# martinber/noaa-apt

Measured on AMD Instinct MI355X. Metric: Msamples/sec WAV->APT-line decode, higher is better.
Workload: dtype f32; 1 GPU; synthetic 48000 Hz APT recording, 600 s (28800000 samples) per GPU, profile=standard: resample 13/50 (959 taps) -> AM envelope -> 37-tap low-pass -> sync correlation + peak picker -> 1198 rows x 2080 px; parallelism=1 GPU(s), 16 independent recordings per GPU and step, no collectives, recordings_per_call=16, mode=strict, rows=1198, n_sync=1199, input_resident_in_hbm=True, distinct_inputs_round_robin=16

## Files before the change

noaa_apt_amd/csrc/apt_capi.hip:

```cpp
#include <cstdio>
#include <cstdlib>
#include <cstring>
#include <memory>
#include <string>

#include "apt_capi_util.hpp"
#include "apt_session.hpp"

namespace {

using namespace apt::capi;

using PlanPtr = std::unique_ptr<aptgpu_plan, apt::capi::PlanDeleter>;


apt::Signal download(const float *d, size_t n, hipStream_t s)
{
    apt::Signal h(n);
    if (n) {
        apt::hip_check(hipMemcpyAsync(h.data(), d, n * sizeof(float), hipMemcpyDeviceToHost, s),
                       "hipMemcpyAsync D2H");
        apt::hip_check(hipStreamSynchronize(s), "hipStreamSynchronize");
    }
    return h;
// ... 189 lines not shown
        (void)hipSetDevice(plan->device);
        plan->sync_all();
        plan->sync_all();
        auto v = plan->timer.collect(plan->stream);
        *n_out = v.size();
        for (size_t i = 0; i < v.size() && i < cap && out; ++i) out[i] = v[i];
        return APTGPU_OK;
    } catch (const Error &) {
        return APTGPU_ERR_HIP;
    }
}

int aptgpu_plan_read_internal(aptgpu_plan *plan, int i, const char *name, void *host_out,
                              size_t bytes, size_t *size_out)
{
    if (!plan || !name || i < 0 || static_cast<size_t>(i) >= plan->last_slots.size())
        return APTGPU_ERR_INVALID;
    aptgpu_plan::Slot &sl = plan->slot_of(i);
    const void *src = nullptr;
    size_t size = 0;
    const std::string n(name);
    if (n == "inv_sinphi") {
        if (size_out) *size_out = sizeof(float);
        if (host_out && bytes >= sizeof(float)) std::memcpy(host_out, &plan->inv_sinphi, sizeof(float));
        return APTGPU_OK;
    }
    if (n == "filtered") { src = sl.filtered.ptr; size = sl.filtered.count * sizeof(float); }
    else if (n == "correlation") { src = sl.correlation.ptr; size = sl.correlation.count * sizeof(float); }
    else if (n == "group_max") { src = sl.gm.ptr; size = sl.gm.count * sizeof(apt::gpu::GroupMax); }
    else if (n == "terminal_words") { src = sl.words.ptr; size = sl.words.count * sizeof(uint64_t); }
    else if (n == "peaks") { src = sl.peaks.ptr; size = sl.peaks.count * sizeof(uint32_t); }
    else if (n == "picker_flags") { src = sl.flags.ptr; size = sl.flags.count * sizeof(uint32_t); }
    else if (n == "eqfloat_thresholds") {
        src = sl.eqfloat_ws.ptr ? apt::gpu::eqfloat_ws_thresholds(sl.eqfloat_ws.ptr) : nullptr;
        size = sl.eqfloat_ws.ptr ? 2 * 255 * sizeof(uint32_t) : 0;
    }
    else return APTGPU_ERR_INVALID;
    if (size_out) *size_out = size;
    (void)hipSetDevice(plan->device);
    try {
        plan->sync_all();
    } catch (const Error &) {
        return APTGPU_ERR_HIP;
    }
    const size_t take = bytes < size ? bytes : size;
    if (take && host_out && src &&
        hipMemcpy(host_out, src, take, hipMemcpyDeviceToHost) != hipSuccess)
        return APTGPU_ERR_HIP;
    return APTGPU_OK;
}

}

namespace apt::capi {

int decode_host(const aptgpu_context *ctx_in, const aptgpu_settings *settings, const float *signal,
                const uint8_t *wav_data, const apt::WavInfo *wav, size_t n, uint32_t input_rate_hz, int sync,
                float **rows_out, size_t *n_out, aptgpu_stats *stats, char *err, size_t err_cap)
{
    *rows_out = nullptr;
// ... 488 lines not shown
```

noaa_apt_amd/csrc/apt_kernels.hpp:

```cpp
#pragma once

#include <hip/hip_runtime.h>

#include <cstdint>

namespace apt::gpu {

struct Result {
    int32_t status;
    int32_t reason;
    uint32_t n_rows;
    uint32_t n_sync;
    uint64_t work_len;
    uint64_t n_out;
};

struct ImageResult {
    int32_t status;
    int32_t reason;
    uint32_t height;
    uint32_t telemetry_row;
    float low, high;
    float telemetry_quality;
    int32_t channel_a, channel_b;
// ... 48 lines not shown
                      uint32_t ntaps, uint32_t l, uint32_t m, float *out, uint64_t w);
uint32_t f16taps_pairs_per_phase(uint32_t l, uint32_t ntaps);
float f16taps_pack(uint32_t l, const float *coeff, uint32_t ntaps, uint16_t *table);
void resample_f16taps(hipStream_t s, const float *x, uint64_t n, const uint16_t *table, uint32_t ntaps,
                      uint32_t l, uint32_t m, float unscale, float *out, uint64_t w);
void fir_decimate(hipStream_t s, const float *x, uint64_t n, const float *coeff, uint32_t ntaps,
                  uint32_t m, float *out, uint64_t n_out);
void demodulate(hipStream_t s, const float *x, uint64_t n, float cosphi2, float sinphi, float *out);
void correlate(hipStream_t s, const float *f, uint64_t n_corr, uint32_t pw, float *corr);
void terminals(hipStream_t s, const float *corr, uint64_t n_corr, uint32_t md, uint64_t *bits);
void orbit_walk(hipStream_t s, const uint64_t *bits, const float *corr, uint64_t n_corr, uint64_t work_len,
                uint32_t spr, uint32_t md, uint32_t *peaks, uint32_t peaks_cap, Result *res);
void gather_rows(hipStream_t s, const float *f, const uint32_t *peaks, Result *res,
                 uint32_t spr, uint32_t pw, bool raw, float *rows, uint32_t rows_cap);
void gather_rows_call(hipStream_t s, const CallArgs &call, const SlotPtrs *d_slots, uint32_t spr, uint32_t pw,
                      uint32_t max_rows_cap, const LaunchSwitches &sw = LaunchSwitches{});

void nosync_rows_call(hipStream_t s, const CallArgs &call, const SlotPtrs *d_slots, uint32_t spr, uint32_t m2, uint64_t max_w);

bool fused_supported(uint32_t l, uint32_t m, uint32_t t1, uint32_t t2, uint32_t pw);
uint32_t fused_group_size(uint32_t l);
bool fused_takes_pcm16(uint32_t l, uint32_t m);
uint32_t fused_tap_table_floats(uint32_t l, uint32_t m, uint32_t t1, int ch);
void fused_branch_taps(uint32_t l, uint32_t m, const float *coeff, uint32_t t1, int ch, float *hs, uint32_t t1_layout = 0);
uint32_t fused_pad_t1(uint32_t l, uint32_t m, uint32_t t1, uint32_t t2, uint32_t pw);
uint32_t fused_pad_t2(uint32_t l, uint32_t m, uint32_t t2, uint32_t pw);
uint32_t fused_phase_pad_t2(uint32_t t2, uint32_t pw);
int fused_chunk_of(uint32_t m, bool fast);
void fused_lowpass_pairs(const float *h2, uint32_t t2, float *h2p);
uint32_t fused_f16_table_dwords(uint32_t l, uint32_t m, uint32_t t1);
float fused_f16_branch_taps(uint32_t l, uint32_t m, const float *coeff, uint32_t t1, uint32_t *table);
bool fused_f16_supported(uint32_t l, uint32_t m, uint32_t t1, uint32_t t2, uint32_t pw);
float fused_gm_slack(uint32_t pw, float scale = 1.f);
// ... 96 lines not shown
```

noaa_apt_amd/csrc/apt_kernels_fused_any_impl.hpp:

```cpp
#pragma once

#include "apt_kernels_fused_any_launch.hpp"
#include "apt_envelope.hpp"
#include "apt_sync_corr.hpp"

#include <atomic>
#include <type_traits>

#pragma clang fp contract(off)

namespace apt::gpu {


namespace {


constexpr int kGS = 52;
constexpr float kNegInfAny = -__builtin_huge_valf();


typedef float f2 __attribute__((ext_vector_type(2)));

template <int KPT>
__host__ __device__ constexpr int pad_ofs(int e)
// ... 220 lines not shown
#pragma unroll
                for (int jj = 0; jj < KPT; ++jj) {
                    if (j0 + jj < G.t2) {
                        const float hj = h2[j0 + jj];
#pragma unroll
                        for (int u = 0; u < KPT; ++u) acc[u] = acc[u] + win[KPT + u - jj] * hj;
                    }
                }
            }
#pragma unroll
            for (int u = 0; u < KPT; ++u) A[P(b0) + u] = acc[u];
        }
    }
    __syncthreads();

    for (uint32_t q = tid * 4; q < G.own; q += NTHR * 4) {
        const uint64_t k = static_cast<uint64_t>(o0) + q;
        const float *src = A + P(static_cast<int>(G.pre + q));
        if (k + 3 < w) {
            *reinterpret_cast<float4 *>(f_out + k) = make_float4(src[0], src[1], src[2], src[3]);
        } else {
            for (int e = 0; e < 4; ++e)
                if (k + e < w) f_out[k + e] = src[e];
        }
    }
    if (gm_out == nullptr) return;

    const uint32_t pw = PWC > 0 ? static_cast<uint32_t>(PWC) : G.pulse / 2u;
    const uint32_t pulse = 2u * pw;
    float *AB = X;
    {
        const int b0 = static_cast<int>(G.pre) + tid * KPT;
        if (b0 < static_cast<int>(G.pre + G.own + 36u * pw)) {
            float bs[KPT];
            if constexpr (PWC > 0) {
                constexpr int NW = KPT + 2 * PWC - 1;
                float wv[NW];
                const float *src = A + P(b0);
// ... 116 lines not shown
```

noaa_apt_amd/csrc/apt_kernels_fused_impl.hpp:

```cpp
#pragma once

#include "apt_kernels_fused_launch.hpp"
#include "apt_envelope.hpp"
#include "apt_sync_corr.hpp"

#include <hip/hip_runtime.h>

#include <algorithm>
#include <atomic>
#include <cmath>
#include <cstdlib>
#include <type_traits>

#pragma clang fp contract(off)

#define APT_S1(n) "s" #n
#define APT_S8_(a, b, c, d, e, f, g, h) APT_S1(a), APT_S1(b), APT_S1(c), APT_S1(d), APT_S1(e), APT_S1(f), APT_S1(g), APT_S1(h)
#define APT_S8(n) APT_S8_X(n)
#define APT_S16(n) APT_S16_X(n)
#define APT_S8_X(n) APT_S8_##n
#define APT_S16_X(n) APT_S16_##n
#define APT_S8_52 APT_S8_(52, 53, 54, 55, 56, 57, 58, 59)
#define APT_S16_36 APT_S8_(36, 37, 38, 39, 40, 41, 42, 43), APT_S8_(44, 45, 46, 47, 48, 49, 50, 51)
#define APT_S16_64 APT_S8_(64, 65, 66, 67, 68, 69, 70, 71), APT_S8_(72, 73, 74, 75, 76, 77, 78, 79)
// ... 1440 lines not shown
                for (int b = 0; b < L; ++b) {
                    const int qi = tid * L + b - static_cast<int>(j);
                    if (kt + b > static_cast<int>(j) && qi >= 0) f[b] = f[b] + Q[qi] * hj;
                }
            }
#pragma unroll
            for (int b = 0; b < L; ++b) P[tid * L + b] = f[b];
            __syncthreads();
        }
    }
    APT_MARK("END f_to_lds");
    if constexpr (APT_FUSED_STOP == 4) return;
    uint32_t slot_late = call.rec[ri].slot;
    asm volatile("" : "+s"(slot_late));
    float *__restrict__ f_out = slots[slot_late].f;
    if (interior) {
        APT_MARK("BEGIN f_store");
        typedef char __attribute__((address_space(1))) *gchar_wptr;
        typedef f4 __attribute__((address_space(1))) *gfloat4_wptr;
        gchar_wptr sb = (gchar_wptr)(f_out + o0);
        const uint32_t voff = static_cast<uint32_t>(tid) * 16u;
#pragma unroll
        for (int e = 0; e * kFusedThreads * 4 < Gm::OWN_K; ++e) {
            const int q = (tid + e * kFusedThreads) * 4;
            if (q < Gm::OWN_K) {
                const float *src = P + Gm::PRE_K + q;
                *(gfloat4_wptr)(sb + voff) = (f4){src[0], src[1], src[2], src[3]};
            }
            sb += kFusedThreads * 16;
            asm volatile("" : "+s"(sb));
        }
        APT_MARK("END f_store");
    } else {
        float *ft = f_out + o0;
        for (int q = tid * 4; q < Gm::OWN_K; q += kFusedThreads * 4) {
            if (Gm::PRE_K + q + 3 < k_hi) {
                const float *src = P + Gm::PRE_K + q;
                *reinterpret_cast<float4 *>(ft + q) = make_float4(src[0], src[1], src[2], src[3]);
            } else {
                for (int e = 0; e < 4; ++e)
                    if (Gm::PRE_K + q + e < k_hi) ft[q + e] = P[Gm::PRE_K + q + e];
            }
        }
    }
    if constexpr (APT_FUSED_STOP == 5) return;
    if (want_gm) {
        GroupMax *__restrict__ gm_out = slots[slot_late].gm;
        constexpr int PUL = 2 * PW;
        static_assert(Gm::GS == 4 * L, "a group is four threads' samples");
        float ab_mine = 0.f;
        {
            APT_MARK("BEGIN pulse_sums");
            int fofs = tid * L;
            int qofs4 = Gm::D_OFF + tid * L;
            int fofs_odd = fofs + 1;
            asm volatile("" : "+v"(fofs), "+v"(fofs_odd), "+v"(qofs4));
            constexpr int NFW = L + PUL - 1;
// ... 283 lines not shown
```

noaa_apt_amd/csrc/apt_kernels_generic.hip:

```cpp
#include "apt_kernels.hpp"
#include "apt_envelope.hpp"

#include <hip/hip_runtime.h>

#include <cstdlib>

#include <cmath>
#include <cstring>
#include <map>
#include <mutex>
#include <tuple>

#pragma clang fp contract(off)

namespace apt::gpu {

namespace {

constexpr int kBlock = 256;

inline unsigned grid_for(uint64_t n, unsigned block, unsigned cap = 256u * 32u)
{
    uint64_t g = (n + block - 1) / block;
    if (g > cap) g = cap;
// ... 233 lines not shown
        res->n_rows = static_cast<uint32_t>(fit - last_fit);
        res->work_len = work_len;
        res->n_out = (fit - last_fit) * 2080u;
        if (len < 5) {
            res->status = 1;
            res->reason = 2;
            res->n_rows = 0;
            res->n_out = 0;
        } else {
            res->status = 0;
            res->reason = 0;
        }
    }
}

__device__ __forceinline__ void gather_rows_body(const float *__restrict__ f, const uint32_t *__restrict__ peaks,
                                                 Result *__restrict__ res, uint32_t spr, uint32_t pw, int raw,
                                                 float *__restrict__ rows, uint32_t rows_cap)
{
    uint32_t n_rows = __hip_atomic_load(&res->n_rows, __ATOMIC_RELAXED, __HIP_MEMORY_SCOPE_AGENT);
    const uint32_t px_per_row = spr / pw;
    if (n_rows > rows_cap) {
        n_rows = rows_cap;
        if (blockIdx.x == 0 && blockIdx.y == 0 && threadIdx.x == 0) {
            __hip_atomic_store(&res->n_rows, rows_cap, __ATOMIC_RELAXED, __HIP_MEMORY_SCOPE_AGENT);
            res->n_out = static_cast<uint64_t>(rows_cap) * px_per_row;
            res->reason = 4;
        }
    }
    const bool quads = (px_per_row & 3u) == 0 && (reinterpret_cast<uintptr_t>(rows) & 15u) == 0;
    for (uint32_t r = blockIdx.y; r < n_rows; r += gridDim.y) {
        const float *src = f + peaks[r];
        float *dst = rows + static_cast<uint64_t>(r) * px_per_row;
        if (quads) {
            for (uint32_t k = blockIdx.x * blockDim.x + threadIdx.x; k < px_per_row / 4u; k += gridDim.x * blockDim.x) {
                const float *p4 = src + static_cast<uint64_t>(4u * k) * pw;
                float4 v = make_float4(p4[0], p4[pw], p4[2u * pw], p4[3u * pw]);
                if (!raw) {
                    v.x = __fadd_rn(0.f, __fmul_rn(v.x, 1.f));
                    v.y = __fadd_rn(0.f, __fmul_rn(v.y, 1.f));
                    v.z = __fadd_rn(0.f, __fmul_rn(v.z, 1.f));
                    v.w = __fadd_rn(0.f, __fmul_rn(v.w, 1.f));
                    if (r == 0 && k == 0) v.x = 0.f;
                }
                *reinterpret_cast<float4 *>(dst + 4u * k) = v;
            }
            continue;
        }
        for (uint32_t c = blockIdx.x * blockDim.x + threadIdx.x; c < px_per_row;
             c += gridDim.x * blockDim.x) {
            float v = src[static_cast<uint64_t>(c) * pw];
            if (!raw) {
                v = __fadd_rn(0.f, __fmul_rn(v, 1.f));
                if (r == 0 && c == 0) v = 0.f;
            }
            dst[c] = v;
        }
    }
}

__global__ void __launch_bounds__(kBlock)
k_gather_rows(const float *__restrict__ f, const uint32_t *__restrict__ peaks,
              Result *__restrict__ res, uint32_t spr, uint32_t pw, int raw,
              float *__restrict__ rows, uint32_t rows_cap)
{
    gather_rows_body(f, peaks, res, spr, pw, raw, rows, rows_cap);
}

__global__ void __launch_bounds__(kBlock)
k_gather_rows_call(const CallArgs call, const SlotPtrs *__restrict__ slots, uint32_t spr, uint32_t pw)
{
    const RecArgs rec = call.rec[blockIdx.z];
    const SlotPtrs sp = slots[rec.slot];
    gather_rows_body(sp.f, sp.peaks, sp.res, spr, pw, 0, rec.rows, rec.rows_cap);
}

template <uint32_t QPR>
__global__ void __launch_bounds__(kBlock)
k_gather_rows_flat(const CallArgs call, const SlotPtrs *__restrict__ slots, uint32_t spr, uint32_t pw)
{
    const RecArgs rec = call.rec[blockIdx.y];
    const SlotPtrs sp = slots[rec.slot];
    Result *__restrict__ res = sp.res;
    uint32_t n_rows = __hip_atomic_load(&res->n_rows, __ATOMIC_RELAXED, __HIP_MEMORY_SCOPE_AGENT);
    if (n_rows > rec.rows_cap) {
        n_rows = rec.rows_cap;
        if (blockIdx.x == 0 && threadIdx.x == 0) {
            __hip_atomic_store(&res->n_rows, rec.rows_cap, __ATOMIC_RELAXED, __HIP_MEMORY_SCOPE_AGENT);
            res->n_out = static_cast<uint64_t>(rec.rows_cap) * (QPR * 4u);
            res->reason = 4;
        }
    }
    const float *__restrict__ f = sp.f;
    const uint32_t *__restrict__ peaks = sp.peaks;
    float *__restrict__ rows = rec.rows;
    const uint32_t total = n_rows * QPR;
    for (uint32_t q = blockIdx.x * kBlock + threadIdx.x; q < total; q += gridDim.x * kBlock) {
        const uint32_t r = q / QPR, k = q - r * QPR;
        const float *p4 = f + peaks[r] + static_cast<uint64_t>(4u * k) * pw;
        float4 v = make_float4(p4[0], p4[pw], p4[2u * pw], p4[3u * pw]);
        v.x = __fadd_rn(0.f, __fmul_rn(v.x, 1.f));
        v.y = __fadd_rn(0.f, __fmul_rn(v.y, 1.f));
        v.z = __fadd_rn(0.f, __fmul_rn(v.z, 1.f));
        v.w = __fadd_rn(0.f, __fmul_rn(v.w, 1.f));
        if (q == 0) v.x = 0.f;
        *reinterpret_cast<float4 *>(rows + static_cast<uint64_t>(q) * 4u) = v;
    }
}

__global__ void k_set_result(Result *res, Result value) { *res = value; }

__global__ void __launch_bounds__(kBlock)
k_nosync_rows_call(const CallArgs call, const SlotPtrs *__restrict__ slots, uint32_t spr, uint32_t m2)
{
    const RecArgs rec = call.rec[blockIdx.y];
    const float *__restrict__ f = slots[rec.slot].f;
    const uint64_t aligned = rec.w / spr * spr;
    uint64_t n_out = aligned / m2;
    if (n_out > rec.rows_cap) n_out = rec.rows_cap;
    const uint64_t stride = static_cast<uint64_t>(gridDim.x) * blockDim.x;
    for (uint64_t k = static_cast<uint64_t>(blockIdx.x) * blockDim.x + threadIdx.x; k < n_out; k += stride) {
        const uint64_t i = k * m2;
        rec.rows[k] = i < 1 ? 0.f : __fadd_rn(0.f, __fmul_rn(f[i], 1.f));
    }
    if (blockIdx.x == 0 && threadIdx.x == 0)
        *slots[rec.slot].res = Result{0 , 0, static_cast<uint32_t>(n_out / 2080u), 0, rec.w, n_out};
}

}

void set_result(hipStream_t s, Result *res, Result value)
{
    hipLaunchKernelGGL(k_set_result, dim3(1), dim3(1), 0, s, res, value);
}

void nosync_rows_call(hipStream_t s, const CallArgs &call, const SlotPtrs *d_slots, uint32_t spr, uint32_t m2, uint64_t max_w)
{
    if (call.count == 0 || spr == 0 || m2 == 0) return;
    const uint64_t n = max_w / m2 + 1;
    hipLaunchKernelGGL(k_nosync_rows_call, dim3(grid_for(n, kBlock), call.count), dim3(kBlock), 0, s, call, d_slots, spr, m2);
}

void resample_generic(hipStream_t s, const float *x, uint64_t n, const float *coeff,
                      uint32_t ntaps, uint32_t l, uint32_t m, float *out, uint64_t w)
{
    if (w == 0) return;
    const uint32_t jlim = 2 * ((ntaps - 1) / 2) + 1;
    hipLaunchKernelGGL(k_resample_generic, dim3(grid_for(w, kBlock)), dim3(kBlock), 0, s, x, n,
                       coeff, jlim, l, m, out, w);
}

uint32_t f16taps_pairs_per_phase(uint32_t l, uint32_t ntaps) { return ((ntaps + l - 1) / l + 1) / 2; }

float f16taps_pack(uint32_t l, const float *coeff, uint32_t ntaps, uint16_t *table)
{
// ... 72 lines not shown
    LaunchSwitches sw;
    if (const char *e = std::getenv("APTGPU_GATHER_ITERS")) sw.gather_iters = std::atoi(e);
    if (const char *e = std::getenv("APTGPU_WORDS_DPP")) sw.words_dpp = e[0] != '0';
    if (const char *e = std::getenv("APTGPU_ORBIT_LDS")) sw.orbit_lds = e[0] != '0';
    if (const char *e = std::getenv("APTGPU_ORBIT_THREADS")) sw.orbit_threads = std::atoi(e);
    if (const char *e = std::getenv("APTGPU_ORBIT_ALG")) sw.orbit_alg = e[0] == '0' ? 0 : 1;
    if (const char *e = std::getenv("APTGPU_GM_SLACK_SCALE")) {
        const float v = std::strtof(e, nullptr);
        if (v >= 1.f) sw.gm_slack_scale = v;
    }
    if (const char *e = std::getenv("APTGPU_FUSED_LDS_PAD")) sw.fused_lds_pad = std::max(0, std::atoi(e));
    return sw;
}

void gather_rows_call(hipStream_t s, const CallArgs &call, const SlotPtrs *d_slots, uint32_t spr, uint32_t pw,
                      uint32_t max_rows_cap, const LaunchSwitches &sw)
{
    if (call.count == 0) return;
    {
        const int iters = sw.gather_iters;
        bool aligned = true;
        for (uint32_t i = 0; i < call.count; ++i) aligned = aligned && (reinterpret_cast<uintptr_t>(call.rec[i].rows) & 15u) == 0;
        if (iters > 0 && spr / pw == 2080u && spr % pw == 0 && aligned && max_rows_cap > 0) {
            const uint64_t quads = static_cast<uint64_t>(max_rows_cap < 32768u ? max_rows_cap : 32768u) * 520u;
            const uint64_t per_wg = static_cast<uint64_t>(kBlock) * static_cast<uint64_t>(iters);
            const unsigned gx = static_cast<unsigned>((quads + per_wg - 1) / per_wg);
            hipLaunchKernelGGL(k_gather_rows_flat<520u>, dim3(gx ? gx : 1, call.count), dim3(kBlock), 0, s, call, d_slots, spr, pw);
            return;
        }
    }
    const unsigned rows_cap = max_rows_cap < 32768u ? max_rows_cap : 32768u;
    const unsigned gy = max_rows_cap == 0 ? 1u : (rows_cap + 7u) / 8u;
    const unsigned gx = (spr / pw + 4 * kBlock - 1) / (4 * kBlock);
    hipLaunchKernelGGL(k_gather_rows_call, dim3(gx ? gx : 1, gy, call.count), dim3(kBlock), 0, s, call, d_slots,
                       spr, pw);
}

void gather_rows(hipStream_t s, const float *f, const uint32_t *peaks, Result *res,
                 uint32_t spr, uint32_t pw, bool raw, float *rows, uint32_t rows_cap)
{
    const unsigned gy = rows_cap == 0 ? 1u : (rows_cap < 4096u ? rows_cap : 4096u);
    const unsigned gx = (spr / pw + 4 * kBlock - 1) / (4 * kBlock);
    hipLaunchKernelGGL(k_gather_rows, dim3(gx ? gx : 1, gy), dim3(kBlock), 0, s, f, peaks, res, spr,
                       pw, raw ? 1 : 0, rows, rows_cap);
}


__global__ void __launch_bounds__(256) k_verify_fast_divide(float c, float rc, uint32_t *bad)
{
    const uint32_t i = blockIdx.x * 256u + threadIdx.x;
// ... 75 lines not shown
```

noaa_apt_amd/csrc/apt_kernels_sync.hip:

```cpp
#include "apt_kernels.hpp"
#include "apt_sync_corr.hpp"

#include <hip/hip_runtime.h>

#include <atomic>

#include <cstdlib>
#include <type_traits>

namespace apt::gpu {

namespace {

constexpr int GS = 52;
constexpr uint64_t kGroupMask = (1ull << GS) - 1;
constexpr float kNegInf = -__builtin_huge_valf();

__global__ void __launch_bounds__(256)
k_group_max(const float *__restrict__ corr, uint64_t n_corr, GroupMax *__restrict__ gm, uint32_t ng)
{
    const uint32_t g = blockIdx.x * blockDim.x + threadIdx.x;
    if (g >= ng) return;
    const uint64_t base = static_cast<uint64_t>(g) * GS;
    float mx = kNegInf;
// ... 167 lines not shown
        const float wm = fmaxf(a[q + 1], a[q + 1 + W - K]);
        s_wm[q] = wm;
        if (g < static_cast<int64_t>(ng) && !(wm > s_hi[q])) s_cand[atomicAdd(&s_ncand, 1u)] = static_cast<uint16_t>(q);
        __syncthreads();
    }

    const uint32_t ncand = s_ncand;
    constexpr int kBatch = NL > 0 ? 4 : 1;
    constexpr int NLR = NL > 0 ? NL : 1;
    constexpr uint16_t kDeferred = 0x8000u;
    float *wa = s_win + static_cast<size_t>(wave) * wlen;
    const uint32_t wneed = GS + 38u * pw - 1u;
    auto eval_group = [&](uint64_t base, bool on) -> float {
        for (uint32_t t = lane; t < wlen; t += 64) {
            const uint64_t j = base + t;
            wa[t] = (t < wneed && j < w) ? fsig[j] : 0.f;
        }
        __builtin_amdgcn_wave_barrier();
        const float v = nodes_eval_window<NL, PWC>(wa, on, lane, pw, fast);
        __builtin_amdgcn_wave_barrier();
        return v;
    };
    auto settle = [&](auto exact_tag, int q, float cv, float c2v, bool in_v) -> bool {
        constexpr bool EXACT = decltype(exact_tag)::value;
        const uint64_t base = static_cast<uint64_t>(gw0 + q) * GS;
        const bool in2 = in_v && base + lane + md < n_corr;
        if (in_v && gw0 + q == 0 && lane == 0 && !(cv > 0.f)) cv = 0.f;
        const unsigned long long nanword = __ballot(in_v && cv != cv) & kGroupMask;
        if (cv != cv) cv = kNegInf;
        float sfx_ex;
        if constexpr (DPP) {
// ... 82 lines not shown
            qv[e] = (ci < ncand) ? s_cand[ci] : -1;
            const int64_t g = gw0 + (qv[e] < 0 ? 0 : qv[e]);
            const uint64_t i = static_cast<uint64_t>(g) * GS + lane;
            inv[e] = qv[e] >= 0 && lane < GS && i < n_corr;
            cv[e] = kNegInf;
            c2v[e] = kNegInf;
            if (corr != nullptr) {
                if (inv[e]) {
                    cv[e] = corr[i];
                    if (i + md < n_corr) c2v[e] = corr[i + md];
                }
            } else if constexpr (NL > 0) {
#pragma unroll
                for (int t = 0; t < NL; ++t) {
                    const uint64_t j = static_cast<uint64_t>(g) * GS + lane + 64u * t;
                    fa[e][t] = (qv[e] >= 0 && lane + 64u * t < wneed && j < w) ? fsig[j] : 0.f;
                }
            }
        }
#pragma unroll
        for (int e = 0; e < kBatch; ++e) {
            if (qv[e] < 0) continue;
            if (corr == nullptr) {
                if constexpr (NL > 0) {
#pragma unroll
                    for (int t = 0; t < NL; ++t)
                        if (lane + 64u * t < wlen) wa[lane + 64 * t] = fa[e][t];
                    __builtin_amdgcn_wave_barrier();
                    cv[e] = nodes_eval_window<NL, PWC>(wa, inv[e], lane, pw, fast);
                    __builtin_amdgcn_wave_barrier();
                } else {
// ... 938 lines not shown
```

noaa_apt_amd/csrc/apt_plan.hip:

```cpp
#include "apt_plan.hpp"

#include <atomic>
#include <cmath>
#include <cstdio>
#include <cstdlib>
#include <cstring>

namespace apt {

void hip_check(hipError_t e, const char *what)
{
    if (e != hipSuccess) {
        throw Error{ErrorKind::Hip, std::string(what) + ": " + hipGetErrorString(e), static_cast<int>(e)};
    }
}

KernelTimer::~KernelTimer()
{
    for (auto &p : pairs_) {
        (void)hipEventDestroy(p.a);
        (void)hipEventDestroy(p.b);
    }
    for (auto e : pool_) (void)hipEventDestroy(e);
}
// ... 306 lines not shown
        Signal lp(plan->taps_lowpass);
        if (plan->fused_pad_t2) {
            lp.resize(plan->fused_pad_t2, 0.f);
            Signal padded(lp);
            padded.resize(lp.size() + 16, 0.f);
            upload(plan->d_taps_lowpass_pad, padded);
        }
        Signal h2p(2 * (lp.size() + 1) + 16, 0.f);
        gpu::fused_lowpass_pairs(lp.data(), static_cast<uint32_t>(lp.size()), h2p.data());
        upload(plan->d_taps_lowpass_pairs, h2p);
    }

    plan->slots.resize(static_cast<size_t>(depth) * static_cast<size_t>(max_batch));
    const uint64_t w = plan->max_work_len;
    for (auto &sl : plan->slots) {
        sl.filtered.alloc(w + 64);
        if (sync) {
            sl.peaks.alloc(plan->max_rows + 2);
            const uint64_t ng = w / gpu::sync_group_size() + 2;
            const uint64_t chunks = ng / gpu::sync_chunk_groups() + 2;
            sl.gm.alloc(ng + 64);
            sl.words.alloc(ng + 64);
            sl.nanw.alloc(ng + 64);
            sl.slot_nt.alloc(chunks * gpu::sync_slot_cap());
            sl.slot_cnt.alloc(chunks);
            sl.orbit_ws.alloc(gpu::sync_orbit_ws_words(w, plan->spr));
            sl.flags.alloc(32);
            hip_check(hipMemsetAsync(sl.flags.ptr, 0, 32 * sizeof(uint32_t), plan->stream), "hipMemset flags");
            if (plan->fused == 0) sl.correlation.alloc(w + 64);
            if (plan->mode == APTGPU_MODE_GENERIC) sl.bits.alloc(w / 64 + plan->md / 64 + 4);
        }
// ... 130 lines not shown
    for (int i = 0; i < count; ++i) last_slots[static_cast<size_t>(i)] = slot0 + i;
    if (user_stream) {
        apt::hip_check(hipEventRecord(ev_user, user_stream), "hipEventRecord");
        apt::hip_check(hipStreamWaitEvent(cur, ev_user, 0), "hipStreamWaitEvent");
    }
    auto timed_on = [&](hipStream_t st, const char *name, auto &&launch) {
        const bool dominant = !std::strcmp(name, "fused_front_end") || !std::strcmp(name, "resample_generic") ||
                              !std::strcmp(name, "resample_f16taps");
        timer.begin(st, name, dominant);
        launch();
        timer.end(st);
    };
    auto timed = [&](const char *name, auto &&launch) { timed_on(cur, name, launch); };

    const bool use_fused = fused != 0 && !keep_steps;
    const bool want_sync = sync && work_is_multiple;
    if (!use_fused && sync) {
        bool grew = false;
        for (int i = 0; i < count; ++i) {
            Slot &sl = slots[static_cast<size_t>(slot0 + i)];
            if (!sl.correlation.ptr) {
                sl.correlation.alloc(max_work_len + 64);
                grew = true;
            }
        }
        if (grew) {
            sync_all();
            upload_slot_table();
        }
    }
// ... 182 lines not shown
#endif
            gather_reps = rep_g;
            for_chunks(live, [&](const CallArgs &c, uint64_t max_w, uint32_t) {
                if (!(skip & 1))
                    for (int r = 0; r < rep_w; ++r)
                        timed("sync_nodes", [&] { sync_nodes(cur, c, d_slots.ptr, max_w, pw, spr, md, use_fused && fused_fast, !use_fused, sw); });
                if (!(skip & 2))
                    for (int r = 0; r < rep_o; ++r)
                        timed("sync_orbit", [&] { sync_orbit(cur, c, d_slots.ptr, spr, md, pw, picker_force, sw); });
            });
            gather_wanted = !(skip & 4);
        }
        if (gather_wanted)
            for (int r = 0; r < gather_reps; ++r)
                for_chunks(live, [&](const CallArgs &c, uint64_t, uint32_t max_cap) {
                    timed("gather_rows", [&] { gather_rows_call(cur, c, d_slots.ptr, spr, pw, max_cap, sw); });
                });
    } else {
        if (l2 == 1 && !keep_steps) {
            for (size_t from = 0; from < live.size(); from += static_cast<size_t>(kMaxCall)) {
                const size_t to = std::min(live.size(), from + static_cast<size_t>(kMaxCall));
                uint64_t max_w = 0;
                uint32_t max_cap = 0;
                CallArgs c = make_call(live, from, to, &max_w, &max_cap);
                for (size_t k = from; k < to; ++k)
                    c.rec[k - from].rows_cap = static_cast<uint32_t>(std::min<uint64_t>(rows_cap_floats[live[k]], 0xFFFFFFFFull));
                timed("final_decimate", [&] { nosync_rows_call(cur, c, d_slots.ptr, spr, m2, max_w); });
            }
        } else
        for (int i : live) {
            Slot &sl = slots[static_cast<size_t>(slot0 + i)];
            const uint64_t w = wlen[static_cast<size_t>(i)];
            const uint64_t aligned = w / spr * spr;
            uint64_t n_out = out_len_nosync(w);
            if (n_out > rows_cap_floats[i]) n_out = rows_cap_floats[i];
            if (l2 > 1 && export_filtered) {
                const uint64_t d0 = apt::fast_resampling_export_geom(aligned, l2, m2, 1).d0;
                timed("final_resample", [&] { resample_at(cur, sl.filtered.ptr, aligned, d_one.ptr, 1, l2, d0, m2, d_rows[i], n_out); });
            } else if (l2 > 1) {
                timed("final_resample", [&] {
                    resample_generic(cur, sl.filtered.ptr, aligned, d_one.ptr, 1, l2, m2, d_rows[i], n_out);
                });
// ... 257 lines not shown
```

noaa_apt_amd/csrc/apt_plan.hpp:

```cpp
#pragma once

#include <hip/hip_runtime.h>

#include <cstdint>
#include <map>
#include <memory>
#include <string>
#include <vector>

#include "../../include/aptgpu.h"
#include "apt_host.hpp"
#include "apt_kernels.hpp"
#include "apt_kernels_color.hpp"
#include "apt_kernels_despeckle.hpp"
#include "apt_kernels_eqfloat.hpp"
#include "apt_kernels_map.hpp"
#include "apt_kernels_png.hpp"
#include "apt_kernels_project.hpp"
#include "apt_wav.hpp"

namespace apt {

void hip_check(hipError_t e, const char *what);

// ... 64 lines not shown
    int device = 0;
    int mode = APTGPU_MODE_STRICT;
    std::vector<hipStream_t> streams;
    hipStream_t stream = nullptr;
    bool front_serial = false;
    std::vector<hipEvent_t> ev_front;
    int prev_front = -1;
    hipStream_t front_stream = nullptr;
    std::vector<hipEvent_t> ev_pre;
    int chain_cus = 0;
    hipStream_t user_stream = nullptr;
    hipEvent_t ev_user = nullptr;
    uint64_t calls = 0;
    int last_stream = 0;
    std::vector<int> last_slots;

    aptgpu_settings settings{};
    uint32_t input_rate = 0;
    bool sync = true;

    uint32_t l = 1, m = 1;
    apt::Signal taps_resample;
    float cosphi2 = 0.f, sinphi = 0.f;
    apt::Signal taps_lowpass;
    uint32_t spr = 0, md = 0, pw = 0, n_sync_taps = 0;
    bool work_is_multiple = false;
    uint32_t l2 = 1, m2 = 1;

    size_t max_samples = 0;
    uint64_t max_work_len = 0;
// ... 126 lines not shown
```

Baseline: 556,400 Msamples/s.

## Store filtered signal in phase-blocked layout so row gather reads contiguously

The fused kernel now writes the filtered envelope in a blocked layout: within each block of pw*32 samples, samples sharing the same phase mod pw sit next to each other. Row gather, nosync decimation and the sync correlation readers all switch to the blocked index, so the strided pw-stride gather becomes contiguous 128-byte reads. The cost is extra index arithmetic and strided LDS reads in the fused store. The sync group evaluation now does scattered reads of the filtered buffer, and a host-side unblocking path is added for debug readback.

```diff
diff --git a/noaa_apt_amd/csrc/apt_capi.hip b/noaa_apt_amd/csrc/apt_capi.hip
--- a/noaa_apt_amd/csrc/apt_capi.hip
+++ b/noaa_apt_amd/csrc/apt_capi.hip
@@ -227,18 +227,25 @@
 int aptgpu_plan_read_internal(aptgpu_plan *plan, int i, const char *name, void *host_out,
                               size_t bytes, size_t *size_out)
 {
-    if (!plan || !name || i < 0 || static_cast<size_t>(i) >= plan->last_slots.size())
-        return APTGPU_ERR_INVALID;
+    if (!plan || !name || i < 0) return APTGPU_ERR_INVALID;
+    const std::string n(name);
+    if (n == "f_block") {
+        const uint32_t v[3] = {plan->pw, apt::gpu::kFBlockK, plan->last_f_blocked ? 1u : 0u};
+        if (size_out) *size_out = sizeof v;
+        if (host_out && bytes) std::memcpy(host_out, v, bytes < sizeof v ? bytes : sizeof v);
+        return APTGPU_OK;
+    }
+    if (static_cast<size_t>(i) >= plan->last_slots.size()) return APTGPU_ERR_INVALID;
     aptgpu_plan::Slot &sl = plan->slot_of(i);
     const void *src = nullptr;
     size_t size = 0;
-    const std::string n(name);
     if (n == "inv_sinphi") {
         if (size_out) *size_out = sizeof(float);
         if (host_out && bytes >= sizeof(float)) std::memcpy(host_out, &plan->inv_sinphi, sizeof(float));
         return APTGPU_OK;
     }
-    if (n == "filtered") { src = sl.filtered.ptr; size = sl.filtered.count * sizeof(float); }
+    const bool unblock = n == "filtered" && plan->last_f_blocked;
+    if (n == "filtered" || n == "filtered_raw") { src = sl.filtered.ptr; size = sl.filtered.count * sizeof(float); }
     else if (n == "correlation") { src = sl.correlation.ptr; size = sl.correlation.count * sizeof(float); }
     else if (n == "group_max") { src = sl.gm.ptr; size = sl.gm.count * sizeof(apt::gpu::GroupMax); }
     else if (n == "terminal_words") { src = sl.words.ptr; size = sl.words.count * sizeof(uint64_t); }
@@ -257,6 +264,18 @@
         return APTGPU_ERR_HIP;
     }
     const size_t take = bytes < size ? bytes : size;
+    if (unblock && take && host_out && src) {
+        const size_t cnt = take / sizeof(float);
+        const uint64_t span = apt::gpu::f_block_alloc(cnt, plan->pw);
+        std::vector<float> raw(static_cast<size_t>(span < sl.filtered.count ? span : sl.filtered.count));
+        if (hipMemcpy(raw.data(), src, raw.size() * sizeof(float), hipMemcpyDeviceToHost) != hipSuccess) return APTGPU_ERR_HIP;
+        float *out = static_cast<float *>(host_out);
+        for (size_t k = 0; k < cnt; ++k) {
+            const uint64_t b = apt::gpu::f_block_index<0>(k, plan->pw);
+            out[k] = b < raw.size() ? raw[static_cast<size_t>(b)] : 0.f;
+        }
+        return APTGPU_OK;
+    }
     if (take && host_out && src &&
         hipMemcpy(host_out, src, take, hipMemcpyDeviceToHost) != hipSuccess)
         return APTGPU_ERR_HIP;
diff --git a/noaa_apt_amd/csrc/apt_f_block.hpp b/noaa_apt_amd/csrc/apt_f_block.hpp
--- /dev/null
+++ b/noaa_apt_amd/csrc/apt_f_block.hpp
@@ -0,0 +1,52 @@
+#pragma once
+
+#include <cstdint>
+
+#ifndef APT_F_BLOCK_K
+#define APT_F_BLOCK_K 32
+#endif
+
+#if defined(__HIPCC__) || defined(__CUDACC__)
+#define APT_F_BLOCK_HD __host__ __device__
+#else
+#define APT_F_BLOCK_HD
+#endif
+
+namespace apt::gpu {
+
+constexpr uint32_t kFBlockK = APT_F_BLOCK_K;
+static_assert(kFBlockK >= 32 && (kFBlockK & (kFBlockK - 1)) == 0, "K is a power of two, at least one 128-byte line");
+constexpr uint32_t f_block_log2(uint32_t v) { return v <= 1 ? 0 : 1 + f_block_log2(v >> 1); }
+constexpr uint32_t kFBlockShift = f_block_log2(kFBlockK);
+
+APT_F_BLOCK_HD inline uint64_t f_block_alloc(uint64_t w, uint32_t pw)
+{
+    const uint64_t bs = static_cast<uint64_t>(pw) * kFBlockK;
+    return (w + bs - 1) / bs * bs;
+}
+
+template <uint32_t PWC = 0>
+APT_F_BLOCK_HD inline uint64_t f_block_index(uint64_t i, uint32_t pw_arg)
+{
+    const uint32_t pw = PWC > 0 ? PWC : pw_arg;
+    const uint32_t bs = pw * kFBlockK;
+    if ((i >> 32) == 0) {
+        const uint32_t i32 = static_cast<uint32_t>(i);
+        const uint32_t blk = i32 / bs, rr = i32 - blk * bs;
+        const uint32_t jj = rr / pw, ph = rr - jj * pw;
+        return static_cast<uint64_t>(blk) * bs + (ph * kFBlockK + jj);
+    }
+    const uint64_t blk = i / bs;
+    const uint32_t rr = static_cast<uint32_t>(i - blk * bs);
+    const uint32_t jj = rr / pw, ph = rr - jj * pw;
+    return blk * bs + (ph * kFBlockK + jj);
+}
+
+template <uint32_t PWC = 0>
+APT_F_BLOCK_HD inline uint64_t f_block_phase_index(uint32_t j, uint32_t ph, uint32_t pw_arg)
+{
+    const uint32_t pw = PWC > 0 ? PWC : pw_arg;
+    return static_cast<uint64_t>(j >> kFBlockShift) * (pw * kFBlockK) + (ph * kFBlockK + (j & (kFBlockK - 1u)));
+}
+
+}
diff --git a/noaa_apt_amd/csrc/apt_kernels.hpp b/noaa_apt_amd/csrc/apt_kernels.hpp
--- a/noaa_apt_amd/csrc/apt_kernels.hpp
+++ b/noaa_apt_amd/csrc/apt_kernels.hpp
@@ -1,4 +1,6 @@
 #pragma once
+
+#include "apt_f_block.hpp"
 
 #include <hip/hip_runtime.h>
 
@@ -86,9 +88,10 @@
 void gather_rows(hipStream_t s, const float *f, const uint32_t *peaks, Result *res,
                  uint32_t spr, uint32_t pw, bool raw, float *rows, uint32_t rows_cap);
 void gather_rows_call(hipStream_t s, const CallArgs &call, const SlotPtrs *d_slots, uint32_t spr, uint32_t pw,
-                      uint32_t max_rows_cap, const LaunchSwitches &sw = LaunchSwitches{});
-
-void nosync_rows_call(hipStream_t s, const CallArgs &call, const SlotPtrs *d_slots, uint32_t spr, uint32_t m2, uint64_t max_w);
+                      uint32_t max_rows_cap, const LaunchSwitches &sw = LaunchSwitches{}, bool f_blocked = false);
+
+void nosync_rows_call(hipStream_t s, const CallArgs &call, const SlotPtrs *d_slots, uint32_t spr, uint32_t m2, uint64_t max_w,
+                      bool f_blocked = false);
 
 bool fused_supported(uint32_t l, uint32_t m, uint32_t t1, uint32_t t2, uint32_t pw);
 uint32_t fused_group_size(uint32_t l);
diff --git a/noaa_apt_amd/csrc/apt_kernels_fused_any_impl.hpp b/noaa_apt_amd/csrc/apt_kernels_fused_any_impl.hpp
--- a/noaa_apt_amd/csrc/apt_kernels_fused_any_impl.hpp
+++ b/noaa_apt_amd/csrc/apt_kernels_fused_any_impl.hpp
@@ -2,6 +2,7 @@
 
 #include "apt_kernels_fused_any_launch.hpp"
 #include "apt_envelope.hpp"
+#include "apt_f_block.hpp"
 #include "apt_sync_corr.hpp"
 
 #include <atomic>
@@ -258,14 +259,18 @@
     }
     __syncthreads();
 
-    for (uint32_t q = tid * 4; q < G.own; q += NTHR * 4) {
-        const uint64_t k = static_cast<uint64_t>(o0) + q;
-        const float *src = A + P(static_cast<int>(G.pre + q));
-        if (k + 3 < w) {
-            *reinterpret_cast<float4 *>(f_out + k) = make_float4(src[0], src[1], src[2], src[3]);
-        } else {
-            for (int e = 0; e < 4; ++e)
-                if (k + e < w) f_out[k + e] = src[e];
+    {
+        const uint32_t pwf = PWC > 0 ? static_cast<uint32_t>(PWC) : G.pulse / 2u;
+        const uint32_t bs = pwf * kFBlockK;
+        const uint64_t blk0 = static_cast<uint64_t>(o0) / bs;
+        const uint32_t r0 = static_cast<uint32_t>(static_cast<uint64_t>(o0) - blk0 * bs);
+        float *__restrict__ fb = f_out + blk0 * bs;
+        const uint64_t left = w > static_cast<uint64_t>(o0) ? w - static_cast<uint64_t>(o0) : 0;
+        const uint32_t q_hi = left < G.own ? static_cast<uint32_t>(left) : G.own;
+        for (uint32_t q = tid; q < q_hi; q += NTHR) {
+            const uint32_t rem = r0 + q, br = rem / bs, rr = rem - br * bs;
+            const uint32_t jj = rr / pwf, ph = rr - jj * pwf;
+            fb[static_cast<uint64_t>(br) * bs + (ph * kFBlockK + jj)] = A[P(static_cast<int>(G.pre + q))];
         }
     }
     if (gm_out == nullptr) return;
diff --git a/noaa_apt_amd/csrc/apt_kernels_fused_impl.hpp b/noaa_apt_amd/csrc/apt_kernels_fused_impl.hpp
--- a/noaa_apt_amd/csrc/apt_kernels_fused_impl.hpp
+++ b/noaa_apt_amd/csrc/apt_kernels_fused_impl.hpp
@@ -2,6 +2,7 @@
 
 #include "apt_kernels_fused_launch.hpp"
 #include "apt_envelope.hpp"
+#include "apt_f_block.hpp"
 #include "apt_sync_corr.hpp"
 
 #include <hip/hip_runtime.h>
@@ -1478,33 +1479,64 @@
     uint32_t slot_late = call.rec[ri].slot;
     asm volatile("" : "+s"(slot_late));
     float *__restrict__ f_out = slots[slot_late].f;
-    if (interior) {
+    constexpr int FK = static_cast<int>(kFBlockK), BS = PW * FK;
+    constexpr int TPB = BS / 4;
+    constexpr int BPP = kFusedThreads / TPB;
+    constexpr bool kWholeBlocks = BPP >= 1 && Gm::OWN_K >= 2 * BS;
+    const uint64_t uo0 = static_cast<uint64_t>(o0);
+    auto store_sample = [&](uint64_t blk_floats, int rr, int q) {
+        const int jj = rr / PW, ph = rr - jj * PW;
+        f_out[blk_floats + static_cast<uint32_t>(ph * FK + jj)] = P[Gm::PRE_K + q];
+    };
+    if (kWholeBlocks && interior) {
         APT_MARK("BEGIN f_store");
         typedef char __attribute__((address_space(1))) *gchar_wptr;
         typedef f4 __attribute__((address_space(1))) *gfloat4_wptr;
-        gchar_wptr sb = (gchar_wptr)(f_out + o0);
-        const uint32_t voff = static_cast<uint32_t>(tid) * 16u;
-#pragma unroll
-        for (int e = 0; e * kFusedThreads * 4 < Gm::OWN_K; ++e) {
-            const int q = (tid + e * kFusedThreads) * 4;
-            if (q < Gm::OWN_K) {
-                const float *src = P + Gm::PRE_K + q;
-                *(gfloat4_wptr)(sb + voff) = (f4){src[0], src[1], src[2], src[3]};
-            }
-            sb += kFusedThreads * 16;
-            asm volatile("" : "+s"(sb));
+        const uint64_t bfirst = (uo0 + static_cast<uint64_t>(BS - 1)) / static_cast<uint64_t>(BS);
+        const int d0 = static_cast<int>(bfirst * static_cast<uint64_t>(BS) - uo0);
+        const int nb = (Gm::OWN_K - d0) / BS;
+        gchar_wptr sb = (gchar_wptr)(f_out + bfirst * static_cast<uint64_t>(BS));
+        {
+            const int bl = tid / TPB, it = tid - bl * TPB;
+            const int ph = it / (FK / 4), qd = it - ph * (FK / 4);
+            const float *src = P + (Gm::PRE_K + d0) + (bl * BS + 4 * qd * PW + ph);
+            const uint32_t voff = static_cast<uint32_t>(bl * BS + ph * FK + 4 * qd) * 4u;
+            const int left = (tid < BPP * TPB ? nb : 0) - bl;
+            constexpr int NPASS = (Gm::OWN_K / BS + BPP - 1) / BPP;
+#pragma unroll
+            for (int e = 0; e < NPASS; ++e) {
+                if (left > e * BPP) {
+                    const float *s4 = src + e * BPP * BS;
+                    *(gfloat4_wptr)(sb + voff) = (f4){s4[0], s4[PW], s4[2 * PW], s4[3 * PW]};
+                }
+                sb += BPP * BS * 4;
+                asm volatile("" : "+s"(sb));
+            }
+        }
+        typedef float __attribute__((address_space(1))) *gfloat_wptr;
+        const gchar_wptr hb = (gchar_wptr)(f_out + (bfirst - 1u) * static_cast<uint64_t>(BS));
+        const int nrest = Gm::OWN_K - nb * BS;
+        auto rest = [&](int t) {
+            const bool head = t < d0;
+            const uint32_t rr = static_cast<uint32_t>(t - d0 + (head ? BS : 0));
+            const uint32_t jj = rr / static_cast<uint32_t>(PW), ph = rr - jj * static_cast<uint32_t>(PW);
+            const uint32_t voff = (static_cast<uint32_t>(head ? 0 : (nb + 1) * BS) + ph * static_cast<uint32_t>(FK) + jj) * 4u;
+            *(gfloat_wptr)(hb + voff) = P[Gm::PRE_K + t + (head ? 0 : nb * BS)];
+        };
+        if constexpr (2 * BS - 2 <= kFusedThreads) {
+            if (tid < nrest) rest(tid);
+        } else {
+#pragma unroll 1
+            for (int t = tid; t < nrest; t += kFusedThreads) rest(t);
         }
         APT_MARK("END f_store");
     } else {
-        float *ft = f_out + o0;
-        for (int q = tid * 4; q < Gm::OWN_K; q += kFusedThreads * 4) {
-            if (Gm::PRE_K + q + 3 < k_hi) {
-                const float *src = P + Gm::PRE_K + q;
-                *reinterpret_cast<float4 *>(ft + q) = make_float4(src[0], src[1], src[2], src[3]);
-            } else {
-                for (int e = 0; e < 4; ++e)
-                    if (Gm::PRE_K + q + e < k_hi) ft[q + e] = P[Gm::PRE_K + q + e];
-            }
+        const uint64_t b0 = uo0 / static_cast<uint64_t>(BS);
+        const int r0 = static_cast<int>(uo0 - b0 * static_cast<uint64_t>(BS));
+        const int q_hi = interior ? Gm::OWN_K : (k_hi - Gm::PRE_K < Gm::OWN_K ? k_hi - Gm::PRE_K : Gm::OWN_K);
+        for (int q = tid; q < q_hi; q += kFusedThreads) {
+            const int rem = r0 + q, br = rem / BS;
+            store_sample((b0 + static_cast<uint64_t>(br)) * static_cast<uint64_t>(BS), rem - br * BS, q);
         }
     }
     if constexpr (APT_FUSED_STOP == 5) return;
diff --git a/noaa_apt_amd/csrc/apt_kernels_generic.hip b/noaa_apt_amd/csrc/apt_kernels_generic.hip
--- a/noaa_apt_amd/csrc/apt_kernels_generic.hip
+++ b/noaa_apt_amd/csrc/apt_kernels_generic.hip
@@ -271,6 +271,7 @@
     }
 }
 
+template <bool BLOCKED>
 __device__ __forceinline__ void gather_rows_body(const float *__restrict__ f, const uint32_t *__restrict__ peaks,
                                                  Result *__restrict__ res, uint32_t spr, uint32_t pw, int raw,
                                                  float *__restrict__ rows, uint32_t rows_cap)
@@ -287,12 +288,17 @@
     }
     const bool quads = (px_per_row & 3u) == 0 && (reinterpret_cast<uintptr_t>(rows) & 15u) == 0;
     for (uint32_t r = blockIdx.y; r < n_rows; r += gridDim.y) {
-        const float *src = f + peaks[r];
+        const uint32_t peak = peaks[r];
+        const float *src = f + peak;
+        const uint32_t j0 = peak / pw, ph = peak - j0 * pw;
+        auto at = [&](uint32_t c) -> float {
+            if constexpr (BLOCKED) return f[f_block_phase_index<0>(j0 + c, ph, pw)];
+            else return src[static_cast<uint64_t>(c) * pw];
+        };
         float *dst = rows + static_cast<uint64_t>(r) * px_per_row;
         if (quads) {
             for (uint32_t k = blockIdx.x * blockDim.x + threadIdx.x; k < px_per_row / 4u; k += gridDim.x * blockDim.x) {
-                const float *p4 = src + static_cast<uint64_t>(4u * k) * pw;
-                float4 v = make_float4(p4[0], p4[pw], p4[2u * pw], p4[3u * pw]);
+                float4 v = make_float4(at(4u * k), at(4u * k + 1u), at(4u * k + 2u), at(4u * k + 3u));
                 if (!raw) {
                     v.x = __fadd_rn(0.f, __fmul_rn(v.x, 1.f));
                     v.y = __fadd_rn(0.f, __fmul_rn(v.y, 1.f));
@@ -306,7 +312,7 @@
         }
         for (uint32_t c = blockIdx.x * blockDim.x + threadIdx.x; c < px_per_row;
              c += gridDim.x * blockDim.x) {
-            float v = src[static_cast<uint64_t>(c) * pw];
+            float v = at(c);
             if (!raw) {
                 v = __fadd_rn(0.f, __fmul_rn(v, 1.f));
                 if (r == 0 && c == 0) v = 0.f;
@@ -321,18 +327,19 @@
               Result *__restrict__ res, uint32_t spr, uint32_t pw, int raw,
               float *__restrict__ rows, uint32_t rows_cap)
 {
-    gather_rows_body(f, peaks, res, spr, pw, raw, rows, rows_cap);
-}
-
+    gather_rows_body<false>(f, peaks, res, spr, pw, raw, rows, rows_cap);
+}
+
+template <bool BLOCKED>
 __global__ void __launch_bounds__(kBlock)
 k_gather_rows_call(const CallArgs call, const SlotPtrs *__restrict__ slots, uint32_t spr, uint32_t pw)
 {
     const RecArgs rec = call.rec[blockIdx.z];
     const SlotPtrs sp = slots[rec.slot];
-    gather_rows_body(sp.f, sp.peaks, sp.res, spr, pw, 0, rec.rows, rec.rows_cap);
-}
-
-template <uint32_t QPR>
+    gather_rows_body<BLOCKED>(sp.f, sp.peaks, sp.res, spr, pw, 0, rec.rows, rec.rows_cap);
+}
+
+template <uint32_t QPR, uint32_t PWB, bool BLK>
 __global__ void __launch_bounds__(kBlock)
 k_gather_rows_flat(const CallArgs call, const SlotPtrs *__restrict__ slots, uint32_t spr, uint32_t pw)
 {
@@ -354,8 +361,17 @@
     const uint32_t total = n_rows * QPR;
     for (uint32_t q = blockIdx.x * kBlock + threadIdx.x; q < total; q += gridDim.x * kBlock) {
         const uint32_t r = q / QPR, k = q - r * QPR;
-        const float *p4 = f + peaks[r] + static_cast<uint64_t>(4u * k) * pw;
-        float4 v = make_float4(p4[0], p4[pw], p4[2u * pw], p4[3u * pw]);
+        float4 v;
+        if constexpr (BLK) {
+            const uint32_t pwc = PWB > 0 ? PWB : pw;
+            const uint32_t peak = peaks[r];
+            const uint32_t j0 = peak / pwc, ph = peak - j0 * pwc, j = j0 + 4u * k;
+            v = make_float4(f[f_block_phase_index<PWB>(j, ph, pw)], f[f_block_phase_index<PWB>(j + 1u, ph, pw)],
+                            f[f_block_phase_index<PWB>(j + 2u, ph, pw)], f[f_block_phase_index<PWB>(j + 3u, ph, pw)]);
+        } else {
+            const float *p4 = f + peaks[r] + static_cast<uint64_t>(4u * k) * pw;
+            v = make_float4(p4[0], p4[pw], p4[2u * pw], p4[3u * pw]);
+        }
         v.x = __fadd_rn(0.f, __fmul_rn(v.x, 1.f));
         v.y = __fadd_rn(0.f, __fmul_rn(v.y, 1.f));
         v.z = __fadd_rn(0.f, __fmul_rn(v.z, 1.f));
@@ -368,7 +384,7 @@
 __global__ void k_set_result(Result *res, Result value) { *res = value; }
 
 __global__ void __launch_bounds__(kBlock)
-k_nosync_rows_call(const CallArgs call, const SlotPtrs *__restrict__ slots, uint32_t spr, uint32_t m2)
+k_nosync_rows_call(const CallArgs call, const SlotPtrs *__restrict__ slots, uint32_t spr, uint32_t m2, int f_blocked)
 {
     const RecArgs rec = call.rec[blockIdx.y];
     const float *__restrict__ f = slots[rec.slot].f;
@@ -378,7 +394,8 @@
     const uint64_t stride = static_cast<uint64_t>(gridDim.x) * blockDim.x;
     for (uint64_t k = static_cast<uint64_t>(blockIdx.x) * blockDim.x + threadIdx.x; k < n_out; k += stride) {
         const uint64_t i = k * m2;
-        rec.rows[k] = i < 1 ? 0.f : __fadd_rn(0.f, __fmul_rn(f[i], 1.f));
+        const uint64_t fi = f_blocked ? f_block_phase_index<0>(static_cast<uint32_t>(k), 0u, m2) : i;
+        rec.rows[k] = i < 1 ? 0.f : __fadd_rn(0.f, __fmul_rn(f[fi], 1.f));
     }
     if (blockIdx.x == 0 && threadIdx.x == 0)
         *slots[rec.slot].res = Result{0 , 0, static_cast<uint32_t>(n_out / 2080u), 0, rec.w, n_out};
@@ -391,11 +408,13 @@
     hipLaunchKernelGGL(k_set_result, dim3(1), dim3(1), 0, s, res, value);
 }
 
-void nosync_rows_call(hipStream_t s, const CallArgs &call, const SlotPtrs *d_slots, uint32_t spr, uint32_t m2, uint64_t max_w)
+void nosync_rows_call(hipStream_t s, const CallArgs &call, const SlotPtrs *d_slots, uint32_t spr, uint32_t m2, uint64_t max_w,
+                      bool f_blocked)
 {
     if (call.count == 0 || spr == 0 || m2 == 0) return;
     const uint64_t n = max_w / m2 + 1;
-    hipLaunchKernelGGL(k_nosync_rows_call, dim3(grid_for(n, kBlock), call.count), dim3(kBlock), 0, s, call, d_slots, spr, m2);
+    hipLaunchKernelGGL(k_nosync_rows_call, dim3(grid_for(n, kBlock), call.count), dim3(kBlock), 0, s, call, d_slots, spr, m2,
+                       f_blocked ? 1 : 0);
 }
 
 void resample_generic(hipStream_t s, const float *x, uint64_t n, const float *coeff,
@@ -498,7 +517,7 @@
 }
 
 void gather_rows_call(hipStream_t s, const CallArgs &call, const SlotPtrs *d_slots, uint32_t spr, uint32_t pw,
-                      uint32_t max_rows_cap, const LaunchSwitches &sw)
+                      uint32_t max_rows_cap, const LaunchSwitches &sw, bool f_blocked)
 {
     if (call.count == 0) return;
     {
@@ -509,15 +528,27 @@
             const uint64_t quads = static_cast<uint64_t>(max_rows_cap < 32768u ? max_rows_cap : 32768u) * 520u;
             const uint64_t per_wg = static_cast<uint64_t>(kBlock) * static_cast<uint64_t>(iters);
             const unsigned gx = static_cast<unsigned>((quads + per_wg - 1) / per_wg);
-            hipLaunchKernelGGL(k_gather_rows_flat<520u>, dim3(gx ? gx : 1, call.count), dim3(kBlock), 0, s, call, d_slots, spr, pw);
+            const dim3 grid(gx ? gx : 1, call.count);
+#define APT_FLAT_LAUNCH(PWB, BLK) \
+    hipLaunchKernelGGL((k_gather_rows_flat<520u, PWB, BLK>), grid, dim3(kBlock), 0, s, call, d_slots, spr, pw)
+            if (!f_blocked) APT_FLAT_LAUNCH(0u, false);
+            else if (pw == 3) APT_FLAT_LAUNCH(3u, true);
+            else if (pw == 4) APT_FLAT_LAUNCH(4u, true);
+            else if (pw == 5) APT_FLAT_LAUNCH(5u, true);
+            else APT_FLAT_LAUNCH(0u, true);
+#undef APT_FLAT_LAUNCH
             return;
         }
     }
     const unsigned rows_cap = max_rows_cap < 32768u ? max_rows_cap : 32768u;
     const unsigned gy = max_rows_cap == 0 ? 1u : (rows_cap + 7u) / 8u;
     const unsigned gx = (spr / pw + 4 * kBlock - 1) / (4 * kBlock);
-    hipLaunchKernelGGL(k_gather_rows_call, dim3(gx ? gx : 1, gy, call.count), dim3(kBlock), 0, s, call, d_slots,
-                       spr, pw);
+    if (f_blocked)
+        hipLaunchKernelGGL(k_gather_rows_call<true>, dim3(gx ? gx : 1, gy, call.count), dim3(kBlock), 0, s, call, d_slots,
+                           spr, pw);
+    else
+        hipLaunchKernelGGL(k_gather_rows_call<false>, dim3(gx ? gx : 1, gy, call.count), dim3(kBlock), 0, s, call, d_slots,
+                           spr, pw);
 }
 
 void gather_rows(hipStream_t s, const float *f, const uint32_t *peaks, Result *res,
diff --git a/noaa_apt_amd/csrc/apt_kernels_sync.hip b/noaa_apt_amd/csrc/apt_kernels_sync.hip
--- a/noaa_apt_amd/csrc/apt_kernels_sync.hip
+++ b/noaa_apt_amd/csrc/apt_kernels_sync.hip
@@ -205,7 +205,7 @@
     auto eval_group = [&](uint64_t base, bool on) -> float {
         for (uint32_t t = lane; t < wlen; t += 64) {
             const uint64_t j = base + t;
-            wa[t] = (t < wneed && j < w) ? fsig[j] : 0.f;
+            wa[t] = (t < wneed && j < w) ? fsig[f_block_index<(PWC > 0 ? PWC : 0)>(j, pw)] : 0.f;
         }
         __builtin_amdgcn_wave_barrier();
         const float v = nodes_eval_window<NL, PWC>(wa, on, lane, pw, fast);
@@ -318,7 +318,7 @@
 #pragma unroll
                 for (int t = 0; t < NL; ++t) {
                     const uint64_t j = static_cast<uint64_t>(g) * GS + lane + 64u * t;
-                    fa[e][t] = (qv[e] >= 0 && lane + 64u * t < wneed && j < w) ? fsig[j] : 0.f;
+                    fa[e][t] = (qv[e] >= 0 && lane + 64u * t < wneed && j < w) ? fsig[f_block_index<(PWC > 0 ? PWC : 0)>(j, pw)] : 0.f;
                 }
             }
         }
diff --git a/noaa_apt_amd/csrc/apt_plan.hip b/noaa_apt_amd/csrc/apt_plan.hip
--- a/noaa_apt_amd/csrc/apt_plan.hip
+++ b/noaa_apt_amd/csrc/apt_plan.hip
@@ -344,7 +344,7 @@
     plan->slots.resize(static_cast<size_t>(depth) * static_cast<size_t>(max_batch));
     const uint64_t w = plan->max_work_len;
     for (auto &sl : plan->slots) {
-        sl.filtered.alloc(w + 64);
+        sl.filtered.alloc((plan->fused != 0 ? gpu::f_block_alloc(w, plan->pw) : w) + 64);
         if (sync) {
             sl.peaks.alloc(plan->max_rows + 2);
             const uint64_t ng = w / gpu::sync_group_size() + 2;
@@ -505,6 +505,7 @@
     auto timed = [&](const char *name, auto &&launch) { timed_on(cur, name, launch); };
 
     const bool use_fused = fused != 0 && !keep_steps;
+    last_f_blocked = use_fused;
     const bool want_sync = sync && work_is_multiple;
     if (!use_fused && sync) {
         bool grew = false;
@@ -717,7 +718,7 @@
         if (gather_wanted)
             for (int r = 0; r < gather_reps; ++r)
                 for_chunks(live, [&](const CallArgs &c, uint64_t, uint32_t max_cap) {
-                    timed("gather_rows", [&] { gather_rows_call(cur, c, d_slots.ptr, spr, pw, max_cap, sw); });
+                    timed("gather_rows", [&] { gather_rows_call(cur, c, d_slots.ptr, spr, pw, max_cap, sw, use_fused); });
                 });
     } else {
         if (l2 == 1 && !keep_steps) {
@@ -728,7 +729,7 @@
                 CallArgs c = make_call(live, from, to, &max_w, &max_cap);
                 for (size_t k = from; k < to; ++k)
                     c.rec[k - from].rows_cap = static_cast<uint32_t>(std::min<uint64_t>(rows_cap_floats[live[k]], 0xFFFFFFFFull));
-                timed("final_decimate", [&] { nosync_rows_call(cur, c, d_slots.ptr, spr, m2, max_w); });
+                timed("final_decimate", [&] { nosync_rows_call(cur, c, d_slots.ptr, spr, m2, max_w, use_fused); });
             }
         } else
         for (int i : live) {
diff --git a/noaa_apt_amd/csrc/apt_plan.hpp b/noaa_apt_amd/csrc/apt_plan.hpp
--- a/noaa_apt_amd/csrc/apt_plan.hpp
+++ b/noaa_apt_amd/csrc/apt_plan.hpp
@@ -102,6 +102,7 @@
     uint64_t calls = 0;
     int last_stream = 0;
     std::vector<int> last_slots;
+    bool last_f_blocked = false;
 
     aptgpu_settings settings{};
     uint32_t input_rate = 0;
```

Result: no change. 561,200 Msamples/s, median of 6 (+0.9%).
